# maxrossi91/moni-align

Measured on AMD Instinct MI355X. Metric: aligned reads/s (whole node), 150 bp SE, mouse-chr19-scale x12-haplotype index, higher is better.
Workload: dtype u64/int32

## Files before the change

moni_align_amd/csrc/align_fast.hip:

```cpp
#pragma once
#include <hip/hip_runtime.h>
#include <stdint.h>

#include "align_core.h"
#include "chain_core.h"
#include "render_core.h"

#define AF_MAX_MEMS 64
#define AF_MAX_ANCH 256
#define AF_MAX_CHAINS 128
#define AF_MAX_CAND 16
#define AF_PLAN_AN 96
#define AF_MAX_READ 512
#define AF_QCAP 256
#define AF_TB 104
#define AF_BLK 52
#define AF_LPASS (AF_TB / AF_BLK)
#define AF_TS 32
#define AF_GBLK 104
#define AF_GPASS 3
#define AF_NBIN 99
#define AF_BIN_SMALL 16u
#define AF_NSMALL 3u
#define AF_BIN_BAND 19u
// ... 930 lines not shown
                    gm = A.mems[k];
                    keep = true;
                    if (A.P.filter_freq) { const double fr = static_cast<double>(gm.occ_cnt) / (double)(size_t)total; if (fr > A.P.freq_thr) keep = false; }
                }
                const unsigned long long bal = __ballot(keep);
                const uint32_t at = n_mems + (uint32_t)__popcll(bal & ((1ull << lane) - 1ull));
                if (keep && at < (uint32_t)WT::MM) {
                    af_mem_t x; x.occ_off = gm.occ_off; x.nocc = gm.occ_cnt; x.len = (uint16_t)gm.len; x.idx = (uint16_t)gm.idx; x.rpos = (uint16_t)gm.rpos; x.mate = (uint8_t)gm.mate; x.pad = 0;
                    L.mem[at] = x;
                }
                if (keep) { tot_len += (unsigned long long)gm.len * gm.occ_cnt; n_anch += gm.occ_cnt; }
                n_mems += (uint32_t)__popcll(bal);
            }
            for (int o = 32; o > 0; o >>= 1) { tot_len += __shfl_xor(tot_len, o); n_anch += __shfl_xor(n_anch, o); }
            if (n_mems > (uint32_t)WT::MM || n_anch > (unsigned long long)WT::MA) too_big = true;
            na = af_uni((uint32_t)n_anch);
            if (!too_big && na > 0) {
                avg = (float)(size_t)tot_len / (size_t)n_anch;
                __syncthreads();
                for (uint32_t x = lane; x < na; x += 64) {
                    uint32_t i = 0, base = 0;
                    while (base + L.mem[i].nocc <= x) { base += L.mem[i].nocc; ++i; }
                    const af_mem_t mi = L.mem[i];
                    L.anch[x] = (A.occs[mi.occ_off + (x - base)] + mi.len - 1) | ((uint64_t)i << 40);
                }
                for (uint32_t i = lane; i < na; i += 64) { L.f[i] = 0; L.msc[i] = 0; L.p[i] = 0; L.t[i] = 0; }
            }
        }
        __syncthreads();
        af_plan_read<WT, LEVEL, GEN>(G, L, g, r_in, off, m, na, avg, fallback, too_big);
    }
}

struct af_runcol_t {
    uint64_t (*node)[64]; int16_t (*fa)[64]; int16_t (*ma)[64]; int8_t (*pa)[64]; uint8_t (*ta)[64]; uint8_t (*sa)[64]; int lane;
    __device__ __forceinline__ long long x(uint32_t k) const { return (long long)(uint32_t)node[k][lane]; }
    __device__ __forceinline__ int32_t y(uint32_t k) const { return (int32_t)((node[k][lane] >> 32) & 1023u); }
    __device__ __forceinline__ int32_t w(uint32_t k) const { return (int32_t)((node[k][lane] >> 42) & 1023u); }
    __device__ __forceinline__ uint32_t mate(uint32_t k) const { return (uint32_t)(node[k][lane] >> 62); }
    __device__ __forceinline__ int32_t f(uint32_t k) const { return fa[k][lane]; }
    __device__ __forceinline__ int32_t msc(uint32_t k) const { return ma[k][lane]; }
    __device__ __forceinline__ int32_t p(uint32_t k) const { return pa[k][lane]; }
    __device__ __forceinline__ int32_t t(uint32_t k) const { return ta[k][lane]; }
    __device__ __forceinline__ void set_f(uint32_t k, int32_t v) { fa[k][lane] = (int16_t)v; }
    __device__ __forceinline__ void set_msc(uint32_t k, int32_t v) { ma[k][lane] = (int16_t)v; }
    __device__ __forceinline__ void set_p(uint32_t k, int32_t v) { pa[k][lane] = (int8_t)v; }
    __device__ __forceinline__ void set_t(uint32_t k, int32_t v) { ta[k][lane] = (uint8_t)v; }
    __device__ __forceinline__ uint32_t start(uint32_t q) const { return sa[q][lane]; }
    __device__ __forceinline__ void set_start(uint32_t q, uint32_t v) { sa[q][lane] = (uint8_t)v; }
};
static_assert(AF_RUN_NODES == af_wave_small_t::MA && AF_RUN_CHAINS == af_wave_small_t::MC && AF_RUN_CHAINS <= AF_CTAB && AF_RUN_NODES <= AF_PLAN_AN, "chain_runs_kernel holds what the small instance holds");
__global__ void __launch_bounds__(64) chain_runs_kernel(const af_args_t G) {
    __shared__ uint64_t s_node[AF_RUN_LEN][64];
    __shared__ int16_t s_f[AF_RUN_LEN][64], s_msc[AF_RUN_LEN][64];
    __shared__ int8_t s_p[AF_RUN_LEN][64];
    __shared__ uint8_t s_t[AF_RUN_LEN][64], s_sj[AF_RUN_LEN][64];
    __shared__ uint32_t s_key[4][AF_RUN_CHAINS], s_ord[4][AF_RUN_CHAINS], s_piece[4][AF_RUN_CHAINS];
    __shared__ uint16_t s_ipos[4][AF_RUN_CHAINS], s_jpos[4][AF_RUN_CHAINS];
    __shared__ lsort::frame s_stack[4][16];
    __shared__ uint8_t s_cnt[4][AF_RUN_CHAINS];
    const af_grp_t<16> g;
    const int lane = threadIdx.x, grp = lane >> 4, slot = lane & 15;
    const ak_args_t& A = G.A;
    const ac_params_t& P = A.P;
    const uint32_t n_work = G.ctr[AFC_L0];
    af_runcol_t C{s_node, s_f, s_msc, s_p, s_t, s_sj, lane};
    uint32_t n_routed = 0;
    for (uint32_t w0 = blockIdx.x * 4u; w0 < n_work; w0 += gridDim.x * 4u) {
        const uint32_t w = w0 + (uint32_t)grp;
        const uint32_t r_in = w < n_work ? G.list0[w] : 0u;
        const af_rstage_t& R = G.rstage[r_in];
        const uint32_t n_runs = w < n_work ? G.rflag[r_in] : 0u;
        const bool mine = (uint32_t)slot < n_runs;
        uint32_t fb = 0, n = 0;
        float avg = 0.f;
        uint64_t xbase = 0;
        if (mine) { fb = R.rs[slot]; n = (uint32_t)R.rs[slot + 1] - fb; avg = R.avg; xbase = R.xbase[slot]; }
        if (n > AF_RUN_LEN) n = AF_RUN_LEN;
        {
            uint64_t v[AF_RUN_LEN];
#pragma unroll
            for (uint32_t q = 0; q < AF_RUN_LEN; ++q) v[q] = q < n ? R.node[fb + q] : 0ull;
#pragma unroll
            for (uint32_t q = 0; q < AF_RUN_LEN; ++q) { s_node[q][lane] = v[q]; s_t[q][lane] = 0; }
        }
        cc_run_dp<int32_t, uint32_t>(C, fb, n, (int32_t)P.max_iter, (uint32_t)P.max_pred, (long long)P.max_dist_x, (int32_t)P.max_dist_y, avg);
        uint32_t ns = 0;
        cc_run_starts(C, fb, n, P.min_chain_score, [&](uint32_t j) { C.set_start(ns++, j); });
        uint32_t nk = 0, n_an = 0;
        cc_run_chains(C, fb, n, ns, P.min_chain_score, P.min_chain_length, [](uint32_t) {},
                      [&](uint32_t j0, int32_t, uint32_t cnt, bool keep) { if (keep) { s_msc[nk++][lane] = (int16_t)(j0 | (cnt << 8)); n_an += cnt; } });
        uint32_t ns_all = ns, an_all = n_an, incl = nk;
        for (int o = 1; o < 16; o <<= 1) { ns_all += (uint32_t)__shfl_xor((int)ns_all, o); an_all += (uint32_t)__shfl_xor((int)an_all, o); }
        for (int o = 1; o < 16; o <<= 1) { const uint32_t up = (uint32_t)__shfl_up((int)incl, o, 16); if (slot >= o) incl += up; }
        const uint32_t nk_all = (uint32_t)__shfl((int)incl, 15, 16);
        const bool routed = n_runs > 0;
        const bool big = routed && (ns_all > AF_RUN_CHAINS || an_all > AF_PLAN_AN);
        const bool go = routed && !big;
        if (go) for (uint32_t c = 0; c < nk; ++c) {
            const uint32_t e = (uint32_t)(uint16_t)s_msc[c][lane], j = e & 0xFFu;
            s_key[grp][incl - nk + c] = ((uint32_t)s_f[j - fb][lane] << 8) | j;
            s_piece[grp][incl - nk + c] = e >> 8;
        }
        __syncthreads();
#pragma unroll
        for (uint32_t q = 0; q < (AF_RUN_CHAINS + 15) / 16; ++q) {
            const uint32_t sidx = (uint32_t)slot + 16u * q;
            if (go && sidx < nk_all) {
                const uint32_t pos = cc_chain_pos(s_key[grp], nk_all, sidx);
                s_ord[grp][pos] = (s_key[grp][sidx] & ~0xFFu) | pos;
                s_cnt[grp][pos] = (uint8_t)s_piece[grp][sidx];
                s_jpos[grp][sidx] = (uint16_t)pos;
            }
        }
        __syncthreads();
        if (go) for (uint32_t c = 0; c < nk; ++c) s_sj[c][lane] = (uint8_t)s_jpos[grp][incl - nk + c];
        __syncthreads();
        if (go && nk_all > 16) af_wave_sort<(AF_RUN_CHAINS + 15) / 16>(g, s_ord[grp], nk_all, s_stack[grp], s_ipos[grp], s_jpos[grp], s_piece[grp], [](const uint32_t& x) { return -(int32_t)(x >> 8); });
        __syncthreads();
        {
            uint32_t an_base = 0;
#pragma unroll
            for (uint32_t q = 0; q < (AF_RUN_CHAINS + 15) / 16; ++q) {
                const uint32_t k = (uint32_t)slot + 16u * q;
                const bool in = go && k < nk_all;
                const uint32_t o = in ? (s_ord[grp][k] & 0xFFu) : 0u;
                const uint32_t cn = in ? (uint32_t)s_cnt[grp][o] : 0u;
                uint32_t inc = cn;
                for (int d = 1; d < 16; d <<= 1) { const uint32_t up = (uint32_t)__shfl_up((int)inc, d, 16); if (slot >= d) inc += up; }
                if (in) { s_ipos[grp][o] = (uint16_t)k; s_jpos[grp][k] = (uint16_t)(an_base + inc - cn); }
                an_base += (uint32_t)__shfl((int)inc, 15, 16);
            }
        }
        __syncthreads();
        if (go) {
            af_ctab_t* const CT = G.ctab + (size_t)r_in * AF_CTAB;
            af_anchor_t* const AN = G.plans[r_in].an;
            for (uint32_t c = 0; c < nk; ++c) {
                const uint32_t e = (uint32_t)(uint16_t)s_msc[c][lane], cnt = e >> 8;
                const uint32_t rank = s_ipos[grp][s_sj[c][lane]], an0 = s_jpos[grp][rank];
                int32_t j = (int32_t)(e & 0xFFu);
                af_anchor_t X;
                uint32_t mate = 0;
                for (uint32_t q = 0; q < cnt; ++q) {
                    const uint64_t nd = s_node[(uint32_t)j - fb][lane];
                    const uint32_t len = (uint32_t)(nd >> 42) & 1023u;
                    X.occ = xbase + (uint32_t)nd - len + 1; X.len = (uint16_t)len; X.idx = (uint16_t)((nd >> 52) & 1023u); X.gap_val = 0; X.gap_kind = AF_GAP_NONE; X.pad = 0;
                    AN[an0 + cnt - 1 - q] = X;
                    mate = (uint32_t)(nd >> 62);
                    j = s_p[(uint32_t)j - fb][lane];
                }
                af_ctab_t E; E.score = (int32_t)(s_ord[grp][rank] >> 8); E.an0 = (uint16_t)an0; E.cnt = (uint8_t)cnt; E.strand = (mate & 2u) ? 1 : 0;
                E.left_ref = ac_seq_off(P, ac_lift(P, X.occ)) + 1;
                CT[rank] = E;
            }
            if (slot == 0) {
                const uint64_t r = A.read_lo + r_in;
                const uint32_t m = (uint32_t)(A.offs[r + 1] - A.offs[r]);
                af_plan_t& PH = G.plans[r_in];
                PH.status = ns_all == 0 ? AF_ST_UNALIGNED : AF_ST_CHAINS; PH.n_cand = 0; PH.n_chains = (uint16_t)nk_all; PH.final_cand = 0; PH.n_alt = 0; PH.pad = 0; PH.score2 = 0;
                PH.ref_pos = PH.ref_len = 0; PH.tb0 = 0; PH.pad2 = 0;
                PH.min_score = A.min_score_of_len[m <= A.max_len ? m : A.max_len];
                G.ntasks[r_in] = 0;
                ++n_routed;
            }
        } else if (big && slot == 0) G.big_list[atomicAdd(&G.ctr[AFC_BIG], 1u)] = r_in;
        __syncthreads();
    }
    for (int o = 32; o > 0; o >>= 1) n_routed += (uint32_t)__shfl_xor((int)n_routed, o);
    if (lane == 0 && n_routed) atomicAdd(&G.ctr[AFC_RUNS], n_routed);
}

struct af_plan_view_t { af_anchor_t* an; moni_dp_task_t* tasks; };
struct af_view_t { af_plan_view_t plan; };
__global__ void __launch_bounds__(256) plan_kernel(const af_args_t G) {
    __shared__ int32_t s_diff[8][256];
    __shared__ uint8_t s_left[AF_CTAB][256];
    const int lane = threadIdx.x;
    const ak_args_t& A = G.A;
    const ac_params_t& P = A.P;
    const uint64_t r_in = (uint64_t)blockIdx.x * 256 + threadIdx.x;
    if (r_in >= A.n_reads) return;
    af_plan_t& PL = G.plans[r_in];
    if (PL.status != AF_ST_CHAINS) return;
    const uint64_t r = A.read_lo + r_in;
    const uint64_t off = A.offs[r];
    const uint32_t m = (uint32_t)(A.offs[r + 1] - off);
    const uint32_t n_chains = PL.n_chains;
    const af_ctab_t* const CT = G.ctab + (size_t)r_in * AF_CTAB;
    const uint32_t t0 = (uint32_t)r_in * AF_MAX_TASKS_READ;
    af_view_t V; V.plan.an = PL.an; V.plan.tasks = G.tasks + t0;
    uint32_t status = AF_ST_CAND, why = AF_WHY_N;
    uint32_t n_diff = 0, n_left = 0, n_cand = 0, n_tasks = 0;
    const uint32_t check_k = P.check_k < 8u ? P.check_k : 8u;
    if (P.check_k > 8u) { status = AF_ST_FALLBACK; why = AF_WHY_CAPACITY; }
    for (uint32_t ci = 0; ci < n_chains && n_diff < check_k && status == AF_ST_CAND; ++ci) {
        const af_ctab_t ch = CT[ci];
        { bool f = false; for (uint32_t q = 0; q < n_diff; ++q) f = f || s_diff[q][lane] == ch.score; if (!f) s_diff[n_diff++][lane] = ch.score; }
        if (P.left_mem_check) {
            bool seen = false;
// ... 1726 lines not shown

__global__ void __launch_bounds__(256) gather_lines_kernel(const uint64_t* __restrict__ pool, const uint64_t* __restrict__ len, const uint64_t* __restrict__ off,
                                                           const uint64_t* __restrict__ pos, uint64_t n_reads, uint8_t* __restrict__ out) {
    const int lane = threadIdx.x & 63;
    const uint64_t wave = ((uint64_t)blockIdx.x * 256 + threadIdx.x) >> 6, n_waves = ((uint64_t)gridDim.x * 256) >> 6;
    for (uint64_t r = wave; r < n_reads; r += n_waves) {
        const uint64_t l = len[r];
        const uint8_t* __restrict__ src = reinterpret_cast<const uint8_t*>(pool + off[r]);
        uint8_t* __restrict__ dst = out + pos[r];
        const uint64_t head = l < 8 ? l : ((8 - (reinterpret_cast<uintptr_t>(dst) & 7)) & 7);
        if ((uint64_t)lane < head) dst[lane] = src[lane];
        const uint64_t words = (l - head) >> 3;
        for (uint64_t k = lane; k < words; k += 64) {
            uint64_t w;
            memcpy(&w, src + head + 8 * k, 8);
            *reinterpret_cast<uint64_t*>(dst + head + 8 * k) = w;
        }
        const uint64_t done = head + 8 * words;
        if (done + lane < l) dst[done + lane] = src[done + lane];
    }
}
__global__ void gather_summary_kernel(const uint64_t* __restrict__ len, const uint64_t* __restrict__ pos, uint64_t n_reads, const unsigned long long* __restrict__ dev_sum,
                                      unsigned long long* __restrict__ out3) {
    if (threadIdx.x == 0 && blockIdx.x == 0) {
        out3[0] = n_reads ? pos[n_reads - 1] + len[n_reads - 1] : 0ull;
        out3[1] = dev_sum[0];
        unsigned long long al = dev_sum[1];
        for (int s = 0; s < 16; ++s) al += dev_sum[8 + 8 * s];
        out3[2] = al;
    }
}

static inline bool af_runs_on() { const char* v = getenv("MONI_AF_RUNS"); return !(v && atoi(v) == 0); }
static inline uint32_t af_wave_max() { const char* v = getenv("MONI_AF_WAVE_MAX"); return v ? (uint32_t)strtoul(v, nullptr, 10) : 96u; }
static inline void af_launch_dp(const af_args_t& G, hipStream_t sx, unsigned dp_grid, unsigned n_cu, uint64_t n_units) {
    if (!(G.dbg & 0x20000u)) hipLaunchKernelGGL(band_tasks_kernel, dim3((unsigned)((G.bin_cap + 255) / 256)), dim3(256), 0, sx, G);
    hipLaunchKernelGGL(af_chunk_kernel, dim3(1), dim3(64), 0, sx, G, (uint32_t)AF_GRP_LARGE, (uint32_t)AF_GRP_WILD);
    hipLaunchKernelGGL((dp_lane_kernel<AF_BLK, AF_QCAP, AF_LPASS>), dim3(dp_grid), dim3(64), 0, sx, G, (uint32_t)AF_GRP_LARGE);
    hipLaunchKernelGGL((dp_lane_kernel<AF_TS, AF_TS, 1>), dim3(dp_grid), dim3(64), 0, sx, G, (uint32_t)AF_GRP_SMALL);
    hipLaunchKernelGGL((dp_band_kernel<AF_BANDW>), dim3(n_cu * 8), dim3(64), 0, sx, G, (uint32_t)AF_GRP_BAND);
    hipLaunchKernelGGL((dp_lane_kernel<AF_BLK, AF_QCAP, AF_LPASS, true>), dim3(dp_grid), dim3(64), 0, sx, G, (uint32_t)AF_GRP_WILD);
    hipLaunchKernelGGL((dp_wave_kernel<AF_BLK, AF_LPASS, 4>), dim3(n_cu * 8), dim3(64), 0, sx, G, (uint32_t)AF_GRP_WILD, (uint32_t)AF_GRP_WILD);
    hipLaunchKernelGGL(global_task_kernel, dim3((unsigned)((n_units + 255) / 256)), dim3(256), 0, sx, G);
    const uint64_t gmax = G.task_cap > n_units * AF_MAX_TASKS_READ ? G.task_cap - n_units * AF_MAX_TASKS_READ : 0;
    if (gmax) hipLaunchKernelGGL(global_band_kernel, dim3((unsigned)((gmax + 255) / 256)), dim3(256), 0, sx, G);
    hipLaunchKernelGGL(af_chunk_kernel, dim3(1), dim3(64), 0, sx, G, (uint32_t)AF_GRP_GLOBAL, (uint32_t)AF_GRP_GWILD);
    hipLaunchKernelGGL((dp_band_kernel<AF_BANDW>), dim3(n_cu * 8), dim3(64), 0, sx, G, (uint32_t)AF_GRP_GBAND);
    hipLaunchKernelGGL((dp_lane_kernel<AF_GBLK, AF_QCAP, AF_GPASS>), dim3(dp_grid), dim3(64), 0, sx, G, (uint32_t)AF_GRP_GLOBAL);
    hipLaunchKernelGGL((dp_lane_kernel<AF_GBLK, AF_QCAP, AF_GPASS, true>), dim3(dp_grid), dim3(64), 0, sx, G, (uint32_t)AF_GRP_GWILD);
    hipLaunchKernelGGL((dp_wave_kernel<AF_GBLK, AF_GPASS, 8>), dim3(n_cu * 8), dim3(64), 0, sx, G, (uint32_t)AF_GRP_GLOBAL, (uint32_t)AF_GRP_GWILD);
}
```

moni_align_amd/csrc/chain_core.h:

```cpp
#pragma once
#include <stdint.h>

#if defined(__HIPCC__) || defined(__CUDACC__)
#define CC_HD __host__ __device__ __forceinline__
#else
#define CC_HD inline
#endif

#define CC_MAX_READ 512
#define CC_NARROW_MAX_DIST (1ll << 28)
#define CC_NARROW_MAX_COUNT (1ll << 30)

CC_HD uint32_t cc_ilog2(uint32_t v) {
#if defined(__HIP_DEVICE_COMPILE__)
    return (uint32_t)(31 - __clz((int)v));
#else
    return (uint32_t)(31 - __builtin_clz(v));
#endif
}

template <class P>
inline bool cc_narrow_ok(const P& p) {
    return p.max_dist_x >= 0 && p.max_dist_x <= CC_NARROW_MAX_DIST && p.max_dist_y >= -CC_NARROW_MAX_DIST && p.max_dist_y <= CC_NARROW_MAX_DIST
        && p.max_iter >= 0 && p.max_iter <= CC_NARROW_MAX_COUNT && p.max_pred >= 0 && p.max_pred <= CC_NARROW_MAX_COUNT;
}

template <class I>
CC_HD bool cc_gain(I x_d, I y_i, I y_j, I w_i, bool same_mate, I max_dist_y, float avg_mem_length, I& gain) {
    const I y_d = y_i - y_j;
    const int32_t l = (int32_t)(y_d > x_d ? (y_d - x_d) : (x_d - y_d));
    const uint32_t ilog_l = l > 0 ? cc_ilog2((uint32_t)l) : 0;
    if (same_mate && (y_j >= y_i || y_d > max_dist_y)) return false;
    const I mn = y_d < x_d ? y_d : x_d;
    const I alpha = mn < w_i ? mn : w_i;
    I beta = 0;
    if (!same_mate) {
        if (x_d == 0) ++beta;
        else { const int c_lin = (int)(l * .01 * avg_mem_length); beta = c_lin < (I)ilog_l ? (I)c_lin : (I)ilog_l; }
    } else {
        beta = l > 0 ? ((I)(.01 * l * avg_mem_length) + (I)ilog_l) >> 1 : 0;
    }
    gain = alpha - beta;
    return true;
}


template <class I, class U, class S>
CC_HD void cc_run_dp(S& s, uint32_t fb, uint32_t n, I max_iter, U max_pred, long long max_dist_x, I max_dist_y, float avg_mem_length) {
    I lb = (I)fb;
    for (uint32_t i = fb; i < fb + n; ++i) {
        const uint32_t ki = i - fb;
        const long long x_i = s.x(ki);
        const I y_i = (I)s.y(ki), w_i = (I)s.w(ki);
        const uint32_t mate_i = s.mate(ki);
        I max_f = w_i, max_j = -1;
        U n_pred = 0;
        if ((U)i - (U)lb > (U)max_iter) lb = (I)i - max_iter;
        for (I j = (I)i - 1; j >= lb; --j) {
            const uint32_t kj = (uint32_t)j - fb;
            const long long x_j = s.x(kj);
            const uint32_t mate_j = s.mate(kj);
            if (mate_i != mate_j && ((mate_i ^ mate_j) != 3)) continue;
            if (x_i > x_j + max_dist_x) { lb = j; continue; }
            I gain;
            if (!cc_gain<I>((I)(x_i - x_j), y_i, (I)s.y(kj), w_i, mate_i == mate_j, max_dist_y, avg_mem_length, gain)) continue;
            const I score = (I)s.f(kj) + gain;
            if (score > max_f) { max_f = score; max_j = j; if (n_pred > 0) --n_pred; }
            else if ((U)(I)s.t(kj) == (U)i && (++n_pred > max_pred)) break;
            const I pj = (I)s.p(kj);
            if (pj > 0) s.set_t((uint32_t)pj - fb, (I)i);
        }
        s.set_f(ki, max_f); s.set_p(ki, max_j);
        I m = max_f;
        if (max_j >= 0) { const I mp = (I)s.msc((uint32_t)max_j - fb); if (mp > max_f) m = mp; }
        s.set_msc(ki, m);
    }
}

// ... 55 lines not shown
```

moni_align_amd/csrc/moni_hip.hip:

```cpp
#include <hip/hip_runtime.h>
#include <fcntl.h>
#include <sys/mman.h>
#include <sys/stat.h>
#include <unistd.h>
#include <cstring>
#include <atomic>
#include <chrono>
#include <rocprim/device/device_scan.hpp>
#include <rocprim/device/device_radix_sort.hpp>

#include <sched.h>
#include <cstdio>
#include <cstdlib>
#include <cstring>
#include <string>
#include <thread>
#include <algorithm>
#include <vector>

#include "../../include/moni_hip.h"
#include "owned_buf.hpp"
#include "image.hpp"
#include "lift_build.hpp"
#include "ref_index_io.hpp"
// ... 1509 lines not shown
                HIPCHK(hipMemsetAsync(S.txt_cur.p, 0, AF_TXT_SHARDS * 8 * sizeof(unsigned long long), sx));
#ifdef AF_PROFILE
                if ((rc = S.prof.ensure(32))) return rc;
                if (k < AK_NSET) HIPCHK(hipMemsetAsync(S.prof.p, 0, 32 * 8, sx));
                G.prof = S.prof.p;
                if (const char* v = getenv("MONI_AF_DBG")) G.dbg = (uint32_t)atoi(v);
                {
                    const size_t pp_stride = (size_t)AFPP_WAVE * ((sub_reads + 63) / 64 + 1) + (size_t)AFPP_READ * (sub_reads + 1);
                    if ((rc = S.prep_prof.ensure(pp_stride * ((n_sub + AK_NSET - 1) / AK_NSET)))) return rc;
                    G.prep_prof = S.prep_prof.p + pp_stride * (k / AK_NSET);
                    HIPCHK(hipMemsetAsync(G.prep_prof, 0, pp_stride * sizeof(unsigned long long), sx));
                }
#endif
#ifdef AF_CUTS
                if (const char* v = getenv("MONI_AF_DBG")) G.dbg = (uint32_t)atoi(v);
#endif
                if (const char* v = getenv("MONI_AF_DBG")) G.dbg |= (uint32_t)atoi(v) & (64u | 65536u | 131072u);
                HIPCHK(hipMemsetAsync(S.ctr.p, 0, AF_NCTR * sizeof(uint32_t), sx));
                const bool l0_mid = c->max_len > 200;
                G.l0_mm = l0_mid ? (uint32_t)af_wave_mid_t::MM : (uint32_t)af_wave_small_t::MM; G.l0_ma = l0_mid ? (uint32_t)af_wave_mid_t::MA : (uint32_t)af_wave_small_t::MA;
                G.ctab = l0_mid ? nullptr : S.ctab.p;
                G.rstage = (G.ctab && af_runs_on() && !(G.dbg & 64) && G.chain_narrow) ? S.rstage.p : nullptr;
#if defined(AF_PROFILE) || defined(AF_CUTS)
                if (G.dbg & (4u | 8u | 16u | 32u | 128u | 256u | 512u | 1024u)) G.rstage = nullptr;
#endif
                G.rflag = S.rflag.p;
                if (G.rstage) HIPCHK(hipMemsetAsync(S.rflag.p, 0, nr, sx));
                hipLaunchKernelGGL(classify_kernel, dim3((unsigned)((nr + 255) / 256)), dim3(256), 0, sx, G);
#define AF_LAUNCH_CP(WT, LEVEL, OCC, grid) do { \
                    if ((G.dbg & 64) || !G.chain_narrow) hipLaunchKernelGGL((chain_plan_kernel<WT, LEVEL, OCC, true>), grid, dim3(64), 0, sx, G); \
                    else hipLaunchKernelGGL((chain_plan_kernel<WT, LEVEL, OCC, false>), grid, dim3(64), 0, sx, G); } while (0)
                if (l0_mid) AF_LAUNCH_CP(af_wave_mid_t, 0, 4, dim3((unsigned)std::min<uint64_t>(nr, (uint64_t)n_cu * 4 * 4)));
                else AF_LAUNCH_CP(af_wave_small_t, 0, 8, dim3((unsigned)std::min<uint64_t>(nr, (uint64_t)n_cu * 4 * 8)));
                if (G.rstage) hipLaunchKernelGGL(chain_runs_kernel, dim3((unsigned)std::min<uint64_t>((nr + 3) / 4, (uint64_t)n_cu * 40)), dim3(64), 0, sx, G);
                AF_LAUNCH_CP(af_wave_t, 1, 3, dim3((unsigned)std::min<uint64_t>(nr, (uint64_t)n_cu * 10)));
                AF_LAUNCH_CP(af_wave_huge_t, 2, 1, dim3((unsigned)std::min<uint64_t>(nr, (uint64_t)n_cu)));
#undef AF_LAUNCH_CP
                HIPCHK(hipGetLastError());
                if (G.ctab) hipLaunchKernelGGL(plan_kernel, dim3((unsigned)((nr + 255) / 256)), dim3(256), 0, sx, G);
                hipLaunchKernelGGL(bin_tasks_kernel, dim3((unsigned)((nr + AF_BT_READS - 1) / AF_BT_READS)), dim3(256), 0, sx, G);
                HIPCHK(hipEventRecord(c->af_ev[3 * k], sx));
                af_launch_dp(G, sx, af_dp_grid, (unsigned)n_cu, nr);
                HIPCHK(hipEventRecord(c->af_ev[3 * k + 1], sx));
                hipLaunchKernelGGL(select_kernel, dim3((unsigned)((nr + 255) / 256)), dim3(256), 0, sx, G);
                hipLaunchKernelGGL(traceback_kernel, dim3((unsigned)((af_tb_cap + 255) / 256)), dim3(256), 0, sx, G);
                HIPCHK(hipEventRecord(c->af_ev[3 * k + 2], sx));
                A.read_list = G.fb_list; A.n_reads_dev = G.fb_n;
                hipStream_t sf = c->fb_stream[k % AK_NSET];
                HIPCHK(hipStreamWaitEvent(sf, c->af_ev[3 * k + 2], 0));
                hipLaunchKernelGGL(align_kernel, dim3((unsigned)ak_waves), dim3(64), 0, sf, A);
                constexpr uint64_t FIN_RENDER_BLOCKS_PER_CU = 96;
                if (gpu_text) {
                    hipLaunchKernelGGL(finish_prep_kernel, dim3((unsigned)std::min<uint64_t>((nr + 63) / 64, (uint64_t)n_cu * 32)), dim3(64), 0, sx, G, S.recipes.p);
                    hipLaunchKernelGGL(finish_render_kernel, dim3((unsigned)std::min<uint64_t>(nr, (uint64_t)n_cu * FIN_RENDER_BLOCKS_PER_CU)), dim3(64), 0, sx, G, (const uint32_t*)S.recipes.p);
                } else hipLaunchKernelGGL(finish_kernel, dim3((unsigned)std::min<uint64_t>((nr + 63) / 64, af_fin_grid)), dim3(64), 0, sx, G);
                HIPCHK(hipMemcpyAsync(c->af_ctr_host.p + AF_NCTR * k, S.ctr.p, AF_NCTR * sizeof(uint32_t), hipMemcpyDeviceToHost, sx));
                HIPCHK(hipEventRecord(c->ak_fin[k], sx));
                HIPCHK(hipStreamWaitEvent(sf, c->ak_fin[k], 0));
                if (inorder) {
                    uint64_t* pos = c->ak_dev_pos.p + r0 + 2 * k;
                    size_t tmp_bytes = 0;
                    if (rocprim::exclusive_scan(nullptr, tmp_bytes, A.dev_len, pos, (uint64_t)0, nr, rocprim::plus<uint64_t>(), sf) != hipSuccess || tmp_bytes > gather_tmp_bytes + 16) return MONI_ENODEV;
                    if (rocprim::exclusive_scan(c->gather_tmp[k % AK_NSET].p, tmp_bytes, A.dev_len, pos, (uint64_t)0, nr, rocprim::plus<uint64_t>(), sf) != hipSuccess) return MONI_ENODEV;
                    hipLaunchKernelGGL(gather_lines_kernel, dim3((unsigned)std::min<uint64_t>((nr + 3) / 4, (uint64_t)n_cu * 8)), dim3(256), 0, sf, (const uint64_t*)A.fmt.txt_pool,
                                       (const uint64_t*)A.dev_len, (const uint64_t*)A.dev_off, (const uint64_t*)pos, nr, reinterpret_cast<uint8_t*>(c->ak_block.p + k * txt_per));
                    hipLaunchKernelGGL(gather_summary_kernel, dim3(1), dim3(64), 0, sf, (const uint64_t*)A.dev_len, (const uint64_t*)pos, nr, (const unsigned long long*)A.dev_sum,
                                       c->ak_dev_sum.p + 160 * k + 150);
// ... 26 lines not shown
                    if (hipEventElapsedTime(&ms, c->af_ev[3 * k + 2], c->ak_fin[k]) == hipSuccess) st.t_k_finish += ms / 1e3;
                }
                {
                    const uint32_t* fc = c->af_ctr_host.p + AF_NCTR * k;
                    unsigned long long cells, rb, cutc, slots; memcpy(&cells, fc + AFC_CELLS, 8); memcpy(&rb, fc + AFC_RBYTES, 8); memcpy(&cutc, fc + AFC_CUTCELLS, 8); memcpy(&slots, fc + AFC_SLOTS, 8);
                    st.dp_cells_cut += cutc; st.dp_slots += slots;
                    any_dirs_ovf_batch = any_dirs_ovf_batch || fc[AFC_DIRS_OVF] != 0;
                    st.dp_tasks += fc[AFC_NT] + (fc[AFC_TASKS] >= (uint32_t)(sub_lo[k + 1] - sub_lo[k]) * AF_MAX_TASKS_READ ? fc[AFC_TASKS] - (uint32_t)(sub_lo[k + 1] - sub_lo[k]) * AF_MAX_TASKS_READ : 0u); st.dp_cells += cells; st.kernel_fallback += fbn[16 * k]; st.dp_ref_bytes += rb;
                    for (int x = 0; x < AF_WHY_N; ++x) why_sum[x] += fc[AFC_WHY + x];
                    runs_routed += fc[AFC_RUNS];
                    if (getenv("MONI_AK_PROFILE")) { unsigned long long du; memcpy(&du, fc + AFC_DIROFF, 8); fprintf(stderr, "  direction bits of sub-batch %llu: %.1f MB used of %.1f MB\n", (unsigned long long)k, du / 1e6, af_dirs_cap / 1e6); }
                    if (getenv("MONI_AK_PROFILE")) fprintf(stderr, "  staged kernels, sub-batch %llu: %u DP tasks, %llu cells, %u traced, %u large + %u small + %u global chunks, %u reads to align_kernel%s; %u of the small instance's %u reads chained by chain_runs_kernel\n",
                                                           (unsigned long long)k, fc[AFC_NT], cells, fc[AFC_TRACED], fc[AFC_NCHUNKS], fc[AFC_NCHUNKS + 1], fc[AFC_NCHUNKS + 2], fbn[16 * k], fc[AFC_DIRS_OVF] ? " (direction bytes overflowed)" : "", fc[AFC_RUNS], fc[AFC_L0]);
                    if (getenv("MONI_AK_PROFILE")) { fprintf(stderr, "    DP problems per bin (16 of the large tile by query length <= 8 13 16 24 32 48 64 .. 160 192 224 256, 3 of the small tile <= 8 16 32, 16 global by query length / 16):"); for (int x = 0; x < AF_NBIN; ++x) fprintf(stderr, " %u", fc[AFC_BINS + x]); fprintf(stderr, "\n"); }
#if defined(AF_CUTS)
                    if (getenv("MONI_AK_PROFILE")) { fprintf(stderr, "    tile problems (extension | gap fill q = t | gap fill q != t) x (band <= 16 | wider | extension with t < q | no bound):"); for (int x = 0; x < 12; ++x) fprintf(stderr, "%s %u", x % 4 == 0 ? " |" : "", fc[180 + x]); fprintf(stderr, "\n"); }
#endif
                    if (getenv("MONI_AK_PROFILE")) { fprintf(stderr, "    global problems by band width / 4 (0-3, 4-7, ... , >= 52):"); for (int x = 0; x < 14; ++x) fprintf(stderr, " %u", fc[AFC_BANDH + x]); fprintf(stderr, "\n"); }
                    if (getenv("MONI_AK_PROFILE")) fprintf(stderr, "    handed over because: long read %u, anchors/seeds %u, chains %u, chains to score %u, chain length %u, DP size %u, overlapping anchors %u, wildcard %u, "
                                                           "loop depends on a score %u, extension short of the query end %u, capacity %u, CIGAR %u\n",
                                                           fc[AFC_WHY + 0], fc[AFC_WHY + 1], fc[AFC_WHY + 2], fc[AFC_WHY + 3], fc[AFC_WHY + 4], fc[AFC_WHY + 5], fc[AFC_WHY + 6], fc[AFC_WHY + 7], fc[AFC_WHY + 8], fc[AFC_WHY + 9], fc[AFC_WHY + 10], fc[AFC_WHY + 11]);
                }
                prof[0] += (double)q[5]; prof[1] += (double)q[6]; prof[2] += (double)q[7]; for (int x = 0; x < 4; ++x) prof[3 + x] += (double)q[10 + x];
                for (int x = 0; x < 8; ++x) hist[x] += (double)q[16 + x];
                for (int x = 0; x < 7; ++x) cyc[x] += (double)q[24 + x];
            }
        }
        if (any_dirs_ovf_batch && c->dirs_scale < 32) c->dirs_scale *= 2;
        static_assert(AF_WHY_N == 12, "moni_align_stats_t::handover_why");
        for (int x = 0; x < AF_WHY_N; ++x) why_out[x] = why_sum[x];
#ifdef AF_PROFILE
        if (n_sub) { unsigned long long pf[32]; for (int x = 0; x < (int)std::min<uint64_t>(n_sub, AK_NSET); ++x) { HIPCHK(hipMemcpy(pf, c->af[x].prof.p, sizeof pf, hipMemcpyDeviceToHost));
            fprintf(stderr, "chain_plan_kernel wave cycles (set %d): load+filter+anchors %.3g, chain %.3g (sort %.3g, dp %.3g, ends+backtrack %.3g), lifts %.3g, plan %.3g, whole read %.3g\n", x,
                    (double)pf[0], (double)pf[1], (double)pf[5], (double)pf[6], (double)pf[7], (double)pf[2], (double)pf[3], (double)pf[4]); } }
        if (gpu_text) for (uint64_t k = 0; k < n_sub; ++k) {
            const uint64_t nr = sub_lo[k + 1] - sub_lo[k];
            if (!nr) continue;
            const size_t pp_stride = (size_t)AFPP_WAVE * ((sub_reads + 63) / 64 + 1) + (size_t)AFPP_READ * (sub_reads + 1);
            const size_t nw = (size_t)std::min<uint64_t>((nr + 63) / 64, (uint64_t)n_cu * 32);
            std::vector<unsigned long long> pp(AFPP_WAVE * nw + AFPP_READ * nr);
            HIPCHK(hipMemcpy(pp.data(), c->af[k % AK_NSET].prep_prof.p + pp_stride * (k / AK_NSET), pp.size() * sizeof(unsigned long long), hipMemcpyDeviceToHost));
            unsigned long long first = ~0ull, last_start = 0, last_end = 0; size_t slow = 0; std::vector<unsigned long long> dur(nw);
            for (size_t w = 0; w < nw; ++w) {
                const unsigned long long* W = pp.data() + AFPP_WAVE * w;
                first = std::min(first, W[0]); last_start = std::max(last_start, W[0]); last_end = std::max(last_end, W[1]); dur[w] = W[1] - W[0];
                if (dur[w] > dur[slow]) slow = w;
            }
            std::vector<unsigned long long> sd(dur); std::sort(sd.begin(), sd.end());
            const unsigned long long* W = pp.data() + AFPP_WAVE * slow;
            fprintf(stderr, "finish_prep_kernel sub-batch %llu (%llu reads, %zu wavefronts): span %.3f ms, last wavefront starts at %.3f ms; wavefront time median %.3f ms, 99 %% %.3f ms, max %.3f ms\n",
                    (unsigned long long)k, (unsigned long long)nr, nw, (last_end - first) / 1e5, (last_start - first) / 1e5, sd[nw / 2] / 1e5, sd[nw * 99 / 100] / 1e5, sd[nw - 1] / 1e5);
            fprintf(stderr, "  slowest wavefront %zu (reads %llu..): starts at %.3f ms, ends at %.3f ms; cycles: stitch %llu, lift %llu, MAPQ + sequences %llu, MD %llu, MD of the unlifted %llu, alternatives %llu\n",
                    slow, (unsigned long long)(sub_lo[k] + 64 * slow), (W[0] - first) / 1e5, (W[1] - first) / 1e5, W[2], W[3], W[4], W[5], W[6], W[7]);
            if (sd[nw - 1] > 4 * sd[nw / 2]) {
                fprintf(stderr, "  its lanes (operations of the CIGAR / of the lifted one / MD items / alternatives / to the host; run hint, runs of the lift):");
                for (size_t l = 0; l < 64 && 64 * slow + l < nr; ++l) { const unsigned long long* R = pp.data() + AFPP_WAVE * nw + AFPP_READ * (64 * slow + l);
                    fprintf(stderr, " [%zu: %llu/%llu/%llu/%llu/%llu; %lld, %llu]", l, R[0] & 0xFFFF, (R[0] >> 16) & 0xFFFF, (R[0] >> 32) & 0xFFFF, (R[0] >> 48) & 0xFF, (R[0] >> 56) & 1, (long long)(int32_t)(uint32_t)R[1], R[1] >> 32); }
                fprintf(stderr, "\n");
            }
        }
#endif
        double ak_sum_ms = c->dp_kernel_ms_accum;
        if (n_sub) { float ms = 0; if (hipEventElapsedTime(&ms, c->ak_begin[0], c->ak_done[n_sub - 1]) == hipSuccess) c->dp_kernel_ms_accum = ms; }
        if (getenv("MONI_AK_PROFILE")) fprintf(stderr, "align_kernel: %.3f ms span (%.3f ms summed) in %llu launches, %llu waves x %d reads in flight; wave cycles: take+chain %.3g, later drives %.3g, DP %.3g; lane cycles in ac_init: load %.3g sort %.3g chain-dp %.3g backtrack %.3g\n", c->dp_kernel_ms_accum, ak_sum_ms, (unsigned long long)n_sub, (unsigned long long)ak_waves, (int)AK_NL, prof[0], prof[1], prof[2], prof[3], prof[4], prof[5], prof[6]);
        if (getenv("MONI_AK_PROFILE")) fprintf(stderr, "DP problems run, by live rows min(qlen,tlen) <=16 / <=32 / <=64 / >64: count %.3g %.3g %.3g %.3g, cells %.3g %.3g %.3g %.3g\n",
                                               hist[0], hist[1], hist[2], hist[3], hist[4], hist[5], hist[6], hist[7]);
        if (getenv("MONI_AK_PROFILE")) fprintf(stderr, "wave cycles inside the DP phase: per-read setup %.3g, memo lookups %.3g, DP by live rows <=16 / <=32 / <=64 / >64: %.3g %.3g %.3g %.3g; 1x1 problems answered in closed form: %.3g\n",
// ... 288 lines not shown
```

Before: 44.80 million.

## Pack chain-run DP columns into registers and batch left-reference lifts in chain_runs_kernel

Moves the per-lane f/msc/p/t/start columns of chain_runs_kernel out of shared memory and into packed 64-bit register words, and reuses s_key and s_ipos in place of s_piece. Shared-memory use per block shrinks, and the kernel now pins occupancy with amdgpu_waves_per_eu and sizes its grid to match. The left-reference lift for each chain is batched two at a time in a new af_left_refs, which issues the pdir and lift-table loads for several chains together so their latency overlaps. This costs extra registers and bit-manipulation work, and fixing the occupancy can cause register spills. Profiling stamps are also added.

```diff
diff --git a/moni_align_amd/csrc/align_fast.hip b/moni_align_amd/csrc/align_fast.hip
--- a/moni_align_amd/csrc/align_fast.hip
+++ b/moni_align_amd/csrc/align_fast.hip
@@ -986,30 +986,121 @@
     }
 }
 
-struct af_runcol_t {
-    uint64_t (*node)[64]; int16_t (*fa)[64]; int16_t (*ma)[64]; int8_t (*pa)[64]; uint8_t (*ta)[64]; uint8_t (*sa)[64]; int lane;
+struct af_runcol_t : cc_packed_run_t {
+    const uint64_t (*node)[64]; int lane;
+    __device__ __forceinline__ af_runcol_t(const uint64_t (*nd)[64], int ln) : node(nd), lane(ln) {}
     __device__ __forceinline__ long long x(uint32_t k) const { return (long long)(uint32_t)node[k][lane]; }
     __device__ __forceinline__ int32_t y(uint32_t k) const { return (int32_t)((node[k][lane] >> 32) & 1023u); }
     __device__ __forceinline__ int32_t w(uint32_t k) const { return (int32_t)((node[k][lane] >> 42) & 1023u); }
     __device__ __forceinline__ uint32_t mate(uint32_t k) const { return (uint32_t)(node[k][lane] >> 62); }
-    __device__ __forceinline__ int32_t f(uint32_t k) const { return fa[k][lane]; }
-    __device__ __forceinline__ int32_t msc(uint32_t k) const { return ma[k][lane]; }
-    __device__ __forceinline__ int32_t p(uint32_t k) const { return pa[k][lane]; }
-    __device__ __forceinline__ int32_t t(uint32_t k) const { return ta[k][lane]; }
-    __device__ __forceinline__ void set_f(uint32_t k, int32_t v) { fa[k][lane] = (int16_t)v; }
-    __device__ __forceinline__ void set_msc(uint32_t k, int32_t v) { ma[k][lane] = (int16_t)v; }
-    __device__ __forceinline__ void set_p(uint32_t k, int32_t v) { pa[k][lane] = (int8_t)v; }
-    __device__ __forceinline__ void set_t(uint32_t k, int32_t v) { ta[k][lane] = (uint8_t)v; }
-    __device__ __forceinline__ uint32_t start(uint32_t q) const { return sa[q][lane]; }
-    __device__ __forceinline__ void set_start(uint32_t q, uint32_t v) { sa[q][lane] = (uint8_t)v; }
 };
+static_assert(AF_RUN_LEN <= CC_PACKED_LEN, "a run's columns are cc_packed_run_t's words");
+
+template <int NL>
+__device__ __forceinline__ void af_left_refs(const ac_params_t& P, const uint64_t (&pos)[NL], uint32_t n, uint64_t (&out)[NL]) {
+    bool on[NL], slow[NL];
+    int same[NL];
+#pragma unroll
+    for (int u = 0; u < NL; ++u) {
+        same[u] = -1;
+#pragma unroll
+        for (int v = u - 1; v >= 0; --v) if (pos[v] == pos[u]) same[u] = v;
+        on[u] = (uint32_t)u < n && same[u] < 0;
+        slow[u] = on[u] && !P.pdir;
+        out[u] = 0;
+    }
+    if (P.pdir) {
+        const uint64_t nb = (P.n_text >> MONI_PDIR_SHIFT) + 1;
+        uint64_t e[NL];
+#pragma unroll
+        for (int u = 0; u < NL; ++u) { uint64_t b = pos[u] >> MONI_PDIR_SHIFT; if (b > nb) b = nb; e[u] = on[u] ? P.pdir[b] : 0ull; }
+        uint64_t nxt[NL], l_second[NL], l_start[NL]; uint32_t last[NL];
+#pragma unroll
+        for (int u = 0; u < NL; ++u) {
+            const uint32_t sid = (uint32_t)e[u];
+            nxt[u] = (on[u] && sid + 1 < P.n_seq) ? P.lift_seqs[sid + 1].start : ~0ull;
+            l_second[u] = l_start[u] = 0; last[u] = 0;
+            if (on[u]) { const moni_lift_seq_t& L = P.lift_seqs[sid]; l_second[u] = L.second; l_start[u] = L.start; last[u] = L.run_off + L.n_runs; }
+        }
+        struct run3_t { uint32_t hap, ref, flags; };
+        run3_t r0[NL], r1[NL];
+#pragma unroll
+        for (int u = 0; u < NL; ++u) {
+            if (on[u] && pos[u] >= nxt[u]) { slow[u] = true; on[u] = false; }
+            const uint32_t k = (uint32_t)(e[u] >> 32);
+            r0[u] = r1[u] = run3_t{0, 0, 0};
+            if (on[u]) {
+                const moni_lift_run_t& Q0 = P.lift_runs[k]; r0[u] = run3_t{Q0.hap, Q0.ref, Q0.flags};
+                if (k + 1 < last[u]) { const moni_lift_run_t& Q1 = P.lift_runs[k + 1]; r1[u] = run3_t{Q1.hap, Q1.ref, Q1.flags}; }
+            }
+        }
+        uint64_t lifted[NL], e2[NL];
+#pragma unroll
+        for (int u = 0; u < NL; ++u) {
+            lifted[u] = 0; e2[u] = 0;
+            if (!on[u]) continue;
+            const uint64_t start = pos[u] - l_start[u];
+            uint32_t k = (uint32_t)(e[u] >> 32);
+            run3_t R = r0[u];
+            if (k + 1 < last[u] && !((uint64_t)r1[u].hap > start)) {
+                R = r1[u]; ++k;
+                while (k + 1 < last[u]) { const moni_lift_run_t& N = P.lift_runs[k + 1]; if ((uint64_t)N.hap > start) break; R = run3_t{N.hap, N.ref, N.flags}; ++k; }
+            }
+            lifted[u] = l_second[u] + (uint64_t)R.ref + ((R.flags & MONI_LIFT_INS) ? 0ull : start - (uint64_t)R.hap);
+            uint64_t b = lifted[u] >> MONI_PDIR_SHIFT; if (b > nb) b = nb;
+            e2[u] = P.pdir[b];
+        }
+        uint64_t nxt2[NL], st2[NL];
+#pragma unroll
+        for (int u = 0; u < NL; ++u) {
+            const uint32_t sid = (uint32_t)e2[u];
+            nxt2[u] = (on[u] && sid + 1 < P.n_seq) ? P.lift_seqs[sid + 1].start : ~0ull;
+            st2[u] = on[u] ? P.lift_seqs[sid].start : 0ull;
+        }
+#pragma unroll
+        for (int u = 0; u < NL; ++u) {
+            if (!on[u]) continue;
+            uint32_t sid = (uint32_t)e2[u];
+            if (lifted[u] >= nxt2[u]) {
+                ++sid;
+                while (sid + 1 < P.n_seq && lifted[u] >= P.lift_seqs[sid + 1].start) ++sid;
+                st2[u] = P.lift_seqs[sid].start;
+            }
+            out[u] = lifted[u] - st2[u];
+        }
+    }
+    bool any_slow = false;
+#pragma unroll
+    for (int u = 0; u < NL; ++u) any_slow = any_slow || slow[u];
+    if (any_slow) {
+#pragma unroll 1
+        for (int u = 0; u < NL; ++u) {
+            bool s = false; uint64_t pv = 0;
+#pragma unroll
+            for (int q = 0; q < NL; ++q) if (u == q) { s = slow[q]; pv = pos[q]; }
+            if (!s) continue;
+            const uint64_t r = ac_seq_off(P, ac_lift(P, pv));
+#pragma unroll
+            for (int q = 0; q < NL; ++q) if (u == q) out[q] = r;
+        }
+    }
+#pragma unroll
+    for (int u = 1; u < NL; ++u) {
+#pragma unroll
+        for (int v = 0; v < u; ++v) if (same[u] == v) out[u] = out[v];
+    }
+}
+
+#ifndef AF_RUNS_OCC
+#define AF_RUNS_OCC 5
+#endif
+#ifndef AF_RUNS_FLIGHT
+#define AF_RUNS_FLIGHT 2
+#endif
 static_assert(AF_RUN_NODES == af_wave_small_t::MA && AF_RUN_CHAINS == af_wave_small_t::MC && AF_RUN_CHAINS <= AF_CTAB && AF_RUN_NODES <= AF_PLAN_AN, "chain_runs_kernel holds what the small instance holds");
-__global__ void __launch_bounds__(64) chain_runs_kernel(const af_args_t G) {
+__global__ void __launch_bounds__(64) __attribute__((amdgpu_waves_per_eu(AF_RUNS_OCC, AF_RUNS_OCC))) chain_runs_kernel(const af_args_t G) {
     __shared__ uint64_t s_node[AF_RUN_LEN][64];
-    __shared__ int16_t s_f[AF_RUN_LEN][64], s_msc[AF_RUN_LEN][64];
-    __shared__ int8_t s_p[AF_RUN_LEN][64];
-    __shared__ uint8_t s_t[AF_RUN_LEN][64], s_sj[AF_RUN_LEN][64];
-    __shared__ uint32_t s_key[4][AF_RUN_CHAINS], s_ord[4][AF_RUN_CHAINS], s_piece[4][AF_RUN_CHAINS];
+    __shared__ uint32_t s_key[4][AF_RUN_CHAINS], s_ord[4][AF_RUN_CHAINS];
     __shared__ uint16_t s_ipos[4][AF_RUN_CHAINS], s_jpos[4][AF_RUN_CHAINS];
     __shared__ lsort::frame s_stack[4][16];
     __shared__ uint8_t s_cnt[4][AF_RUN_CHAINS];
@@ -1018,9 +1109,9 @@
     const ak_args_t& A = G.A;
     const ac_params_t& P = A.P;
     const uint32_t n_work = G.ctr[AFC_L0];
-    af_runcol_t C{s_node, s_f, s_msc, s_p, s_t, s_sj, lane};
     uint32_t n_routed = 0;
     for (uint32_t w0 = blockIdx.x * 4u; w0 < n_work; w0 += gridDim.x * 4u) {
+        AF_STAMP(q0);
         const uint32_t w = w0 + (uint32_t)grp;
         const uint32_t r_in = w < n_work ? G.list0[w] : 0u;
         const af_rstage_t& R = G.rstage[r_in];
@@ -1031,19 +1122,17 @@
         uint64_t xbase = 0;
         if (mine) { fb = R.rs[slot]; n = (uint32_t)R.rs[slot + 1] - fb; avg = R.avg; xbase = R.xbase[slot]; }
         if (n > AF_RUN_LEN) n = AF_RUN_LEN;
-        {
-            uint64_t v[AF_RUN_LEN];
-#pragma unroll
-            for (uint32_t q = 0; q < AF_RUN_LEN; ++q) v[q] = q < n ? R.node[fb + q] : 0ull;
-#pragma unroll
-            for (uint32_t q = 0; q < AF_RUN_LEN; ++q) { s_node[q][lane] = v[q]; s_t[q][lane] = 0; }
-        }
+#pragma unroll
+        for (uint32_t q = 0; q < AF_RUN_LEN; ++q) s_node[q][lane] = q < n ? R.node[fb + q] : 0ull;
+        af_runcol_t C(s_node, lane);
+        AF_STAMP(q1); AF_PROF(G, 16, q0, q1);
         cc_run_dp<int32_t, uint32_t>(C, fb, n, (int32_t)P.max_iter, (uint32_t)P.max_pred, (long long)P.max_dist_x, (int32_t)P.max_dist_y, avg);
         uint32_t ns = 0;
         cc_run_starts(C, fb, n, P.min_chain_score, [&](uint32_t j) { C.set_start(ns++, j); });
         uint32_t nk = 0, n_an = 0;
         cc_run_chains(C, fb, n, ns, P.min_chain_score, P.min_chain_length, [](uint32_t) {},
-                      [&](uint32_t j0, int32_t, uint32_t cnt, bool keep) { if (keep) { s_msc[nk++][lane] = (int16_t)(j0 | (cnt << 8)); n_an += cnt; } });
+                      [&](uint32_t j0, int32_t, uint32_t cnt, bool keep) { if (keep) { C.set_msc(nk++, (int32_t)(j0 | (cnt << 8))); n_an += cnt; } });
+        AF_STAMP(q2); AF_PROF(G, 17, q1, q2);
         uint32_t ns_all = ns, an_all = n_an, incl = nk;
         for (int o = 1; o < 16; o <<= 1) { ns_all += (uint32_t)__shfl_xor((int)ns_all, o); an_all += (uint32_t)__shfl_xor((int)an_all, o); }
         for (int o = 1; o < 16; o <<= 1) { const uint32_t up = (uint32_t)__shfl_up((int)incl, o, 16); if (slot >= o) incl += up; }
@@ -1052,9 +1141,9 @@
         const bool big = routed && (ns_all > AF_RUN_CHAINS || an_all > AF_PLAN_AN);
         const bool go = routed && !big;
         if (go) for (uint32_t c = 0; c < nk; ++c) {
-            const uint32_t e = (uint32_t)(uint16_t)s_msc[c][lane], j = e & 0xFFu;
-            s_key[grp][incl - nk + c] = ((uint32_t)s_f[j - fb][lane] << 8) | j;
-            s_piece[grp][incl - nk + c] = e >> 8;
+            const uint32_t e = (uint32_t)(uint16_t)C.msc(c), j = e & 0xFFu;
+            s_key[grp][incl - nk + c] = ((uint32_t)C.f(j - fb) << 8) | j;
+            s_ipos[grp][incl - nk + c] = (uint16_t)(e >> 8);
         }
         __syncthreads();
 #pragma unroll
@@ -1063,14 +1152,14 @@
             if (go && sidx < nk_all) {
                 const uint32_t pos = cc_chain_pos(s_key[grp], nk_all, sidx);
                 s_ord[grp][pos] = (s_key[grp][sidx] & ~0xFFu) | pos;
-                s_cnt[grp][pos] = (uint8_t)s_piece[grp][sidx];
+                s_cnt[grp][pos] = (uint8_t)s_ipos[grp][sidx];
                 s_jpos[grp][sidx] = (uint16_t)pos;
             }
         }
         __syncthreads();
-        if (go) for (uint32_t c = 0; c < nk; ++c) s_sj[c][lane] = (uint8_t)s_jpos[grp][incl - nk + c];
+        if (go) for (uint32_t c = 0; c < nk; ++c) C.set_start(c, (uint32_t)s_jpos[grp][incl - nk + c]);
         __syncthreads();
-        if (go && nk_all > 16) af_wave_sort<(AF_RUN_CHAINS + 15) / 16>(g, s_ord[grp], nk_all, s_stack[grp], s_ipos[grp], s_jpos[grp], s_piece[grp], [](const uint32_t& x) { return -(int32_t)(x >> 8); });
+        if (go && nk_all > 16) af_wave_sort<(AF_RUN_CHAINS + 15) / 16>(g, s_ord[grp], nk_all, s_stack[grp], s_ipos[grp], s_jpos[grp], s_key[grp], [](const uint32_t& x) { return -(int32_t)(x >> 8); });
         __syncthreads();
         {
             uint32_t an_base = 0;
@@ -1087,26 +1176,51 @@
             }
         }
         __syncthreads();
+        AF_STAMP(q3); AF_PROF(G, 18, q2, q3);
+#ifdef AF_PROFILE
+        long long t_out = 0;
+#endif
         if (go) {
             af_ctab_t* const CT = G.ctab + (size_t)r_in * AF_CTAB;
             af_anchor_t* const AN = G.plans[r_in].an;
-            for (uint32_t c = 0; c < nk; ++c) {
-                const uint32_t e = (uint32_t)(uint16_t)s_msc[c][lane], cnt = e >> 8;
-                const uint32_t rank = s_ipos[grp][s_sj[c][lane]], an0 = s_jpos[grp][rank];
-                int32_t j = (int32_t)(e & 0xFFu);
-                af_anchor_t X;
-                uint32_t mate = 0;
-                for (uint32_t q = 0; q < cnt; ++q) {
-                    const uint64_t nd = s_node[(uint32_t)j - fb][lane];
-                    const uint32_t len = (uint32_t)(nd >> 42) & 1023u;
-                    X.occ = xbase + (uint32_t)nd - len + 1; X.len = (uint16_t)len; X.idx = (uint16_t)((nd >> 52) & 1023u); X.gap_val = 0; X.gap_kind = AF_GAP_NONE; X.pad = 0;
-                    AN[an0 + cnt - 1 - q] = X;
-                    mate = (uint32_t)(nd >> 62);
-                    j = s_p[(uint32_t)j - fb][lane];
-                }
-                af_ctab_t E; E.score = (int32_t)(s_ord[grp][rank] >> 8); E.an0 = (uint16_t)an0; E.cnt = (uint8_t)cnt; E.strand = (mate & 2u) ? 1 : 0;
-                E.left_ref = ac_seq_off(P, ac_lift(P, X.occ)) + 1;
-                CT[rank] = E;
+            for (uint32_t c0 = 0; c0 < nk; c0 += AF_RUNS_FLIGHT) {
+                uint64_t lpos[AF_RUNS_FLIGHT]; uint32_t meta[AF_RUNS_FLIGHT];
+#pragma unroll
+                for (int u = 0; u < AF_RUNS_FLIGHT; ++u) { lpos[u] = 0; meta[u] = 0; }
+                const uint32_t nb = nk - c0 < AF_RUNS_FLIGHT ? nk - c0 : (uint32_t)AF_RUNS_FLIGHT;
+                AF_STAMP(a0);
+#pragma unroll 1
+                for (uint32_t u = 0; u < nb; ++u) {
+                    const uint32_t c = c0 + u;
+                    const uint32_t e = (uint32_t)(uint16_t)C.msc(c), cnt = e >> 8;
+                    const uint32_t rank = s_ipos[grp][C.start(c)], an0 = s_jpos[grp][rank];
+                    int32_t j = (int32_t)(e & 0xFFu);
+                    af_anchor_t X;
+                    uint32_t mate = 0;
+                    for (uint32_t q = 0; q < cnt; ++q) {
+                        const uint64_t nd = s_node[(uint32_t)j - fb][lane];
+                        const uint32_t len = (uint32_t)(nd >> 42) & 1023u;
+                        X.occ = xbase + (uint32_t)nd - len + 1; X.len = (uint16_t)len; X.idx = (uint16_t)((nd >> 52) & 1023u); X.gap_val = 0; X.gap_kind = AF_GAP_NONE; X.pad = 0;
+                        AN[an0 + cnt - 1 - q] = X;
+                        mate = (uint32_t)(nd >> 62);
+                        j = C.p((uint32_t)j - fb);
+                    }
+                    const uint32_t mt = rank | (an0 << 8) | (cnt << 16) | ((mate & 2u) << 23);
+#pragma unroll
+                    for (int q = 0; q < AF_RUNS_FLIGHT; ++q) if (u == (uint32_t)q) { lpos[q] = X.occ; meta[q] = mt; }
+                }
+#ifdef AF_PROFILE
+                t_out += clock64() - a0;
+#endif
+                uint64_t lref[AF_RUNS_FLIGHT];
+                af_left_refs<AF_RUNS_FLIGHT>(P, lpos, nb, lref);
+#pragma unroll
+                for (int u = 0; u < AF_RUNS_FLIGHT; ++u) if ((uint32_t)u < nb) {
+                    const uint32_t rank = meta[u] & 0xFFu;
+                    af_ctab_t E; E.score = (int32_t)(s_ord[grp][rank] >> 8); E.an0 = (uint16_t)((meta[u] >> 8) & 0xFFu); E.cnt = (uint8_t)((meta[u] >> 16) & 0xFFu); E.strand = (uint8_t)(meta[u] >> 24);
+                    E.left_ref = lref[u] + 1;
+                    CT[rank] = E;
+                }
             }
             if (slot == 0) {
                 const uint64_t r = A.read_lo + r_in;
@@ -1120,6 +1234,9 @@
             }
         } else if (big && slot == 0) G.big_list[atomicAdd(&G.ctr[AFC_BIG], 1u)] = r_in;
         __syncthreads();
+#ifdef AF_PROFILE
+        { AF_STAMP(q4); t_out = __shfl(t_out, 0); AF_PROF(G, 19, 0, t_out); AF_PROF(G, 20, q3 + t_out, q4); AF_PROF(G, 21, q0, q4); }
+#endif
     }
     for (int o = 32; o > 0; o >>= 1) n_routed += (uint32_t)__shfl_xor((int)n_routed, o);
     if (lane == 0 && n_routed) atomicAdd(&G.ctr[AFC_RUNS], n_routed);
@@ -2912,6 +3029,11 @@
 }
 
 static inline bool af_runs_on() { const char* v = getenv("MONI_AF_RUNS"); return !(v && atoi(v) == 0); }
+static inline unsigned af_runs_grid(uint64_t n_reads, unsigned n_cu) {
+    const char* v = getenv("MONI_AF_RUNS_GRID");
+    const uint64_t want = v ? strtoull(v, nullptr, 10) : 0, groups = (n_reads + 3) / 4;
+    return (unsigned)std::max<uint64_t>(1, std::min<uint64_t>(groups, want ? want : (uint64_t)n_cu * 4 * AF_RUNS_OCC));
+}
 static inline uint32_t af_wave_max() { const char* v = getenv("MONI_AF_WAVE_MAX"); return v ? (uint32_t)strtoul(v, nullptr, 10) : 96u; }
 static inline void af_launch_dp(const af_args_t& G, hipStream_t sx, unsigned dp_grid, unsigned n_cu, uint64_t n_units) {
     if (!(G.dbg & 0x20000u)) hipLaunchKernelGGL(band_tasks_kernel, dim3((unsigned)((G.bin_cap + 255) / 256)), dim3(256), 0, sx, G);
diff --git a/moni_align_amd/csrc/chain_core.h b/moni_align_amd/csrc/chain_core.h
--- a/moni_align_amd/csrc/chain_core.h
+++ b/moni_align_amd/csrc/chain_core.h
@@ -44,6 +44,29 @@
     return true;
 }
 
+
+#define CC_PACKED_LEN 8
+struct cc_packed_run_t {
+    uint64_t f_lo = 0, f_hi = 0, m_lo = 0, m_hi = 0, p_w = 0, t_w = 0, s_w = 0;
+    static CC_HD uint32_t get16(uint64_t lo, uint64_t hi, uint32_t k) { return (uint32_t)((k < 4u ? lo : hi) >> ((k & 3u) << 4)) & 0xFFFFu; }
+    static CC_HD void put16(uint64_t& lo, uint64_t& hi, uint32_t k, uint32_t v) {
+        const uint32_t sh = (k & 3u) << 4;
+        const uint64_t keep = ~(0xFFFFull << sh), val = (uint64_t)(v & 0xFFFFu) << sh;
+        if (k < 4u) lo = (lo & keep) | val; else hi = (hi & keep) | val;
+    }
+    static CC_HD uint32_t get8(uint64_t w, uint32_t k) { return (uint32_t)(w >> (k << 3)) & 0xFFu; }
+    static CC_HD void put8(uint64_t& w, uint32_t k, uint32_t v) { const uint32_t sh = k << 3; w = (w & ~(0xFFull << sh)) | ((uint64_t)(v & 0xFFu) << sh); }
+    CC_HD int32_t f(uint32_t k) const { return (int32_t)(int16_t)get16(f_lo, f_hi, k); }
+    CC_HD int32_t msc(uint32_t k) const { return (int32_t)(int16_t)get16(m_lo, m_hi, k); }
+    CC_HD int32_t p(uint32_t k) const { return (int32_t)(int8_t)get8(p_w, k); }
+    CC_HD int32_t t(uint32_t k) const { return (int32_t)get8(t_w, k); }
+    CC_HD uint32_t start(uint32_t q) const { return get8(s_w, q); }
+    CC_HD void set_f(uint32_t k, int32_t v) { put16(f_lo, f_hi, k, (uint32_t)v); }
+    CC_HD void set_msc(uint32_t k, int32_t v) { put16(m_lo, m_hi, k, (uint32_t)v); }
+    CC_HD void set_p(uint32_t k, int32_t v) { put8(p_w, k, (uint32_t)v); }
+    CC_HD void set_t(uint32_t k, int32_t v) { put8(t_w, k, (uint32_t)v); }
+    CC_HD void set_start(uint32_t q, uint32_t v) { put8(s_w, q, v); }
+};
 
 template <class I, class U, class S>
 CC_HD void cc_run_dp(S& s, uint32_t fb, uint32_t n, I max_iter, U max_pred, long long max_dist_x, I max_dist_y, float avg_mem_length) {
diff --git a/moni_align_amd/csrc/moni_hip.hip b/moni_align_amd/csrc/moni_hip.hip
--- a/moni_align_amd/csrc/moni_hip.hip
+++ b/moni_align_amd/csrc/moni_hip.hip
@@ -1565,7 +1565,7 @@
                     else hipLaunchKernelGGL((chain_plan_kernel<WT, LEVEL, OCC, false>), grid, dim3(64), 0, sx, G); } while (0)
                 if (l0_mid) AF_LAUNCH_CP(af_wave_mid_t, 0, 4, dim3((unsigned)std::min<uint64_t>(nr, (uint64_t)n_cu * 4 * 4)));
                 else AF_LAUNCH_CP(af_wave_small_t, 0, 8, dim3((unsigned)std::min<uint64_t>(nr, (uint64_t)n_cu * 4 * 8)));
-                if (G.rstage) hipLaunchKernelGGL(chain_runs_kernel, dim3((unsigned)std::min<uint64_t>((nr + 3) / 4, (uint64_t)n_cu * 40)), dim3(64), 0, sx, G);
+                if (G.rstage) hipLaunchKernelGGL(chain_runs_kernel, dim3(af_runs_grid(nr, (unsigned)n_cu)), dim3(64), 0, sx, G);
                 AF_LAUNCH_CP(af_wave_t, 1, 3, dim3((unsigned)std::min<uint64_t>(nr, (uint64_t)n_cu * 10)));
                 AF_LAUNCH_CP(af_wave_huge_t, 2, 1, dim3((unsigned)std::min<uint64_t>(nr, (uint64_t)n_cu)));
 #undef AF_LAUNCH_CP
@@ -1658,7 +1658,9 @@
 #ifdef AF_PROFILE
         if (n_sub) { unsigned long long pf[32]; for (int x = 0; x < (int)std::min<uint64_t>(n_sub, AK_NSET); ++x) { HIPCHK(hipMemcpy(pf, c->af[x].prof.p, sizeof pf, hipMemcpyDeviceToHost));
             fprintf(stderr, "chain_plan_kernel wave cycles (set %d): load+filter+anchors %.3g, chain %.3g (sort %.3g, dp %.3g, ends+backtrack %.3g), lifts %.3g, plan %.3g, whole read %.3g\n", x,
-                    (double)pf[0], (double)pf[1], (double)pf[5], (double)pf[6], (double)pf[7], (double)pf[2], (double)pf[3], (double)pf[4]); } }
+                    (double)pf[0], (double)pf[1], (double)pf[5], (double)pf[6], (double)pf[7], (double)pf[2], (double)pf[3], (double)pf[4]);
+            fprintf(stderr, "chain_runs_kernel wave cycles (set %d): header+nodes %.3g, dp+starts+chains %.3g, ranks+sort %.3g, anchors out %.3g, lifts+table %.3g, whole iteration %.3g\n", x,
+                    (double)pf[16], (double)pf[17], (double)pf[18], (double)pf[19], (double)pf[20], (double)pf[21]); } }
         if (gpu_text) for (uint64_t k = 0; k < n_sub; ++k) {
             const uint64_t nr = sub_lo[k + 1] - sub_lo[k];
             if (!nr) continue;
```

After: 44.48 million. No clear change (-0.7%).
